# ParBLiSS/FastANI

Hardware: NVIDIA H100
Metric: genome-pairs/sec (many-to-many, k=16, fragLen=3000) (higher is better)
Workload: dtype u64

## Files before the change

### fastani_b200/csrc/capi.cu

```cuda
#include "common.cuh"
#include <algorithm>
#include <cstring>
#include <cstdlib>

struct bani_ctx    { bani::Ctx c; };
struct bani_genome { bani::Genome g; };
struct bani_index  { bani::Index *ix; };
struct bani_qsketch { bani::QSketch *qs; };

namespace bani {
static thread_local std::string g_err;
void set_last_error(const std::string &m) { g_err = m; }
const char *const PATH_NAMES[NPATH] = {
  "l1.class0", "l1.class1", "l1.class2", "l1.class3", "l1.class4", "l1.class5", "l1.class6", "l1.class7", "l1.class8",
  "l1.class9", "l1.class10", "l1.class11", "l1.class12", "l1.device_wide",
  "lookup.walk_saturated", "lookup.walk_full_bucket",
  "l2.events_nt64", "l2.events_nt128", "l2.events_nt256", "l2.dir1024", "l2.dir4096", "l2.staged", "l2.direct",
  "l2.exact_at_bounds", "l2.exact_total",
  "piece.mapped", "piece.split_hits", "piece.split_events", "cgi.passes", "cgi.sparse"};
}

using namespace bani;

#define BANI_TRY try {
#define BANI_CATCH } catch (const bani::Error &e) { bani::set_last_error(e.what()); return e.code; } \
  catch (const std::bad_alloc &) { bani::set_last_error("host allocation failed"); return BANI_ERR_NOMEM; } \
  catch (const std::exception &e) { bani::set_last_error(e.what()); return BANI_ERR_INTERNAL; }

template <typename T>
static T *host_copy(const std::vector<T> &v)
{
  if (v.empty()) return nullptr;
  T *p = (T *)malloc(sizeof(T) * v.size());
// ... 72 lines not shown
  c->c.prm = *p;
  if (c->c.prm.kmer_size < 1 || c->c.prm.kmer_size > 32) fail(BANI_ERR_LIMIT, "k-mer size %d outside [1, 32]", c->c.prm.kmer_size);
  if (c->c.prm.frag_len < 1) fail(BANI_ERR_ARG, "fragment length must be positive");
  if (c->c.prm.window_size <= 0)
    c->c.prm.window_size = stat_recommended_window_size(p->p_value, p->kmer_size, p->perc_identity, p->frag_len, p->reference_size);
  cudaDeviceProp prop;
  BANI_CUDA(cudaGetDeviceProperties(&prop, device));
  c->c.smCount = prop.multiProcessorCount;
  c->c.memTotal = prop.totalGlobalMem;
  {
    CtxFlags &f = c->c.flags;
    if (getenv("BANI_NO_SKETCH_REUSE")) f.sketchReuse = 0;
    if (const char *e = getenv("BANI_MAX_HITS_PER_PIECE")) f.maxHitsPerPiece = std::max(1ll, atoll(e));
    if (const char *e = getenv("BANI_FRAG_L1_MAX")) f.fragL1Max = std::max(0ll, atoll(e));
    if (const char *e = getenv("BANI_L2_STAGE")) f.l2Stage = atoi(e) != 0;
    if (const char *e = getenv("BANI_TRACE")) f.trace = atoi(e) != 0;
    if (const char *e = getenv("BANI_L2E_BUCKETS")) { const int v = atoi(e); if (v == 1024 || v == 4096) f.l2eBuckets = v; }
    if (const char *e = getenv("BANI_CGI_SPARSE")) {
      const std::string v(e);
      if (v == "-1") f.cgiSparse = -1;
      else if (v == "0") f.cgiSparse = 0;
      else if (v == "1") f.cgiSparse = 1;
      else fail(BANI_ERR_ARG, "BANI_CGI_SPARSE=%s is not -1 (chosen per piece), 0 (dense) or 1 (sparse)", e);
    }
    uint64_t b = 0;
    if (const char *e = getenv("BANI_INDEX_BUDGET")) {
      if (!parse_byte_count(e, &b)) fail(BANI_ERR_ARG, "BANI_INDEX_BUDGET=%s is not a byte count (digits, optionally followed by K, M or G)", e);
      f.indexBytesBudget = b;
    }
    if (const char *e = getenv("BANI_QUERY_BUDGET")) {
// ... 40 lines not shown
  return BANI_OK;
  BANI_CATCH
}

int bani_ctx_set_flag(bani_ctx *ctx, const char *name, int64_t value)
{
  BANI_TRY
  if (!ctx || !name) fail(BANI_ERR_ARG, "null argument");
  CtxFlags &f = ctx->c.flags;
  const std::string n(name);
  if (n == "sketch_reuse") f.sketchReuse = value != 0;
  else if (n == "max_hits_per_piece") { if (value < 1) fail(BANI_ERR_ARG, "max_hits_per_piece must be positive"); f.maxHitsPerPiece = value; }
  else if (n == "frag_l1_max") { if (value < 0) fail(BANI_ERR_ARG, "frag_l1_max must not be negative"); f.fragL1Max = value; }
  else if (n == "l2e_buckets") { if (value != 0 && value != 1024 && value != 4096) fail(BANI_ERR_ARG, "l2e_buckets must be 0, 1024 or 4096"); f.l2eBuckets = (int)value; }
  else if (n == "l2_stage") f.l2Stage = value != 0;
  else if (n == "upload_group_words") { if (value < 1) fail(BANI_ERR_ARG, "upload_group_words must be positive"); f.uploadGroupWords = value; }
  else if (n == "frags_per_piece") { if (value < 1 || value > (1ll << 18)) fail(BANI_ERR_ARG, "frags_per_piece must be in [1, 2^18]"); f.fragsPerPiece = value; }
  else if (n == "event_bytes_per_piece") { if (value < 0) fail(BANI_ERR_ARG, "event_bytes_per_piece must not be negative"); f.eventBytesPerPiece = value; }
  else if (n == "cgi_table_queries") { if (value < 0) fail(BANI_ERR_ARG, "cgi_table_queries must not be negative"); f.cgiTableQueries = value; }
  else if (n == "l2_fast") f.l2Fast = value != 0;
  else if (n == "count_paths") f.countPaths = value != 0;
  else if (n == "cgi_sparse") { if (value < -1 || value > 1) fail(BANI_ERR_ARG, "cgi_sparse must be -1, 0 or 1"); f.cgiSparse = (int)value; }
  else if (n == "index_bytes_budget") { if (value < 0) fail(BANI_ERR_ARG, "index_bytes_budget must not be negative"); f.indexBytesBudget = (unsigned long long)value; }
  else if (n == "query_sketch_budget") { if (value < 0) fail(BANI_ERR_ARG, "query_sketch_budget must not be negative"); f.querySketchBudget = (unsigned long long)value; }
  else fail(BANI_ERR_ARG, "unknown flag '%s'", name);
  return BANI_OK;
  BANI_CATCH
}

int bani_ctx_path_counts(bani_ctx *ctx, char (*names)[32], uint64_t *counts, int32_t n_max, int32_t *n)
// ... 694 lines not shown
```

### fastani_b200/csrc/common.cuh

```cuda
#pragma once
#include <cuda_runtime.h>
#include <stdint.h>
#include <string>
#include <vector>
#include <memory>
#include <map>
#include <stdexcept>
#include <cstdio>
#include <cstdarg>
#include <chrono>
#include "../../include/fastani_b200.h"

namespace bani {

struct Error : std::runtime_error {
  int code;
  Error(int c, const std::string &m) : std::runtime_error(m), code(c) {}
};

void set_last_error(const std::string &m);

[[noreturn]] inline void fail(int code, const char *fmt, ...)
{
  char buf[512];
// ... 135 lines not shown
};

template <typename T>
struct View {
  T *p = nullptr; size_t n = 0;
  size_t bytes() const { return n * sizeof(T); }
  void release() {}
};

struct CtxFlags {
  int sketchReuse = 1;
  long long maxHitsPerPiece = 3ll << 29;
  long long fragL1Max = 8192;
  int l2eBuckets = 0;
  int trace = 0;
  int l2Stage = 1;
  long long uploadGroupWords = 16ll << 20;
  long long fragsPerPiece = 1ll << 18;
  long long eventBytesPerPiece = 0;
  long long cgiTableQueries = 0;
  int l2Fast = 1;
  int countPaths = 0;
  int cgiSparse = -1;
  unsigned long long indexBytesBudget = 0;
  unsigned long long querySketchBudget = 0;
};

enum PathId {
  P_L1_CLASS0 = 0, P_L1_DEVICE_WIDE = 13,
  P_LOOKUP_WALK_SATURATED, P_LOOKUP_WALK_FULL_BUCKET,
  P_L2_EVENTS_NT64, P_L2_EVENTS_NT128, P_L2_EVENTS_NT256, P_L2_DIR1024, P_L2_DIR4096, P_L2_STAGED, P_L2_DIRECT,
  P_L2_EXACT_AT_BOUNDS, P_L2_EXACT_TOTAL,
  P_PIECE_MAPPED, P_PIECE_SPLIT_HITS, P_PIECE_SPLIT_EVENTS, P_CGI_PASSES, P_CGI_SPARSE,
  NPATH
};
extern const char *const PATH_NAMES[NPATH];

struct Ctx {
  int device = 0;
  cudaStream_t stream = nullptr;
  cudaStream_t copyStream = nullptr;
  bani_params prm{};
  CtxFlags flags;
  int smCount = 0;
  size_t memTotal = 0;
  StatLut lut;
  DevBuf<int32_t> d_minHits; DevBuf<uint32_t> d_rowOff; DevBuf<float> d_ident, d_upper;
// ... 130 lines not shown
void qsketch_map(Ctx *ctx, const Index *ix, const QSketch *const *sketches, int32_t nSketches,
                 bool wantRows, bool wantCgi, MapOutput &out, bool wantFrags = false);

static constexpr unsigned long long FRAG_L1_MAX = 8192;
static constexpr int FRAG_NCLASS = 13;
static_assert(P_L1_DEVICE_WIDE == FRAG_NCLASS, "one path counter per L1 size class");
__host__ __device__ inline int frag_class_items(int cls)
{
  return cls < 8 ? cls + 1 : (cls == 8 ? 10 : cls == 9 ? 12 : cls == 10 ? 16 : cls == 11 ? 24 : 32);
}
struct FragL1Args {
  const uint32_t *segStart; const int32_t *sCount; int32_t F;
  const uint32_t *hitLo, *hitCnt; const unsigned long long *hitOff;
  const uint32_t *posIdx; const int2 *recPos;
  const int32_t *minHits; int fragLen, keyBits;
  int32_t *stSeq, *stStart, *stEnd;
  uint32_t *candCount;
};
void frag_classify(Ctx *ctx, const uint32_t *segStart, const unsigned long long *hitOff, int32_t F,
                   uint32_t *candCount, uint32_t *fragClass, uint32_t *classCount, uint32_t *classList, unsigned long long maxFast);
void frag_l1_fast(Ctx *ctx, const FragL1Args &a, const uint32_t *classList, const uint32_t *classCount);
void cand_stage(Ctx *ctx, const int32_t *cFrag, const int32_t *cSeq, const int32_t *cStart, const int32_t *cEnd, uint32_t C,
                const uint32_t *segStart, const unsigned long long *hitOff, int32_t *stSeq, int32_t *stStart, int32_t *stEnd,
                uint32_t *candCount);
void cand_compact(Ctx *ctx, const uint32_t *segStart, const unsigned long long *hitOff, int32_t F,
                  const uint32_t *candCount, const uint32_t *candOff, const int32_t *stSeq, const int32_t *stStart,
                  const int32_t *stEnd, int32_t *cFrag, int32_t *cSeq, int32_t *cStart, int32_t *cEnd);

void synth_genome(Ctx *ctx, uint64_t seed, uint32_t ancestor, uint32_t strain, uint32_t ppm,
                  int64_t len, uint8_t *hostOut);

size_t cub_sort_pairs_u32_temp(size_t n);
void   cub_sort_pairs_u32(void *temp, size_t tempBytes, const uint32_t *kin, uint32_t *kout,
                          const uint32_t *vin, uint32_t *vout, size_t n, int endBit, cudaStream_t s);
size_t cub_sort_keys_u64_temp(size_t n);
void   cub_sort_keys_u64(void *temp, size_t tempBytes, const uint64_t *kin, uint64_t *kout, size_t n,
                         int beginBit, int endBit, cudaStream_t s);
size_t cub_sort_pairs_u64_u32_temp(size_t n);
void   cub_sort_pairs_u64_u32(void *temp, size_t tempBytes, const uint64_t *kin, uint64_t *kout,
                              const uint32_t *vin, uint32_t *vout, size_t n, int endBit, cudaStream_t s);
size_t cub_scan_u32_temp(size_t n);
void   cub_exclusive_sum_u32(void *temp, size_t tempBytes, const uint32_t *in, uint32_t *out, size_t n, cudaStream_t s);
// ... 5 lines not shown
```

### fastani_b200/csrc/hits.cu

```cuda
#define BANI_FILE_TAG 1
#include "common.cuh"

namespace bani {

static inline unsigned nblk(uint64_t n, int t = 256) { return (unsigned)((n + t - 1) / t); }

__global__ void frag_classify_kernel(const uint32_t *segStart, const unsigned long long *hitOff, int32_t F,
                                     uint32_t *candCount, uint32_t *fragClass, uint32_t *classCount, uint32_t *classList, unsigned long long maxFast)
{
  const int f = blockIdx.x * blockDim.x + threadIdx.x;
  if (f >= F) return;
  const unsigned long long n = hitOff[segStart[f + 1]] - hitOff[segStart[f]];
  candCount[f] = 0;
  uint32_t cls = FRAG_NCLASS + 1;
  if (n > maxFast) cls = FRAG_NCLASS;
  else if (n > 0) { cls = 0; while (n > 256ull * (unsigned long long)frag_class_items(cls)) cls++; }
  fragClass[f] = cls;
  if (cls <= FRAG_NCLASS) { const uint32_t o = atomicAdd(&classCount[cls], 1u); if (cls < FRAG_NCLASS) classList[(size_t)cls * F + o] = (uint32_t)f; }
}

template <int ITEMS, int DB>
__device__ __forceinline__ uint32_t *block_radix_sort(uint32_t *in, uint32_t *out, uint16_t *hist ,
                                                       uint32_t *digitBase , uint32_t *wsum , int keyBits)
{
// ... 84 lines not shown
  const uint32_t *sorted = block_radix_sort<ITEMS, DB>(bufA, bufB, hist, digitBase, wsum, a.keyBits);
  uint32_t keys[ITEMS];
#pragma unroll
  for (int i = 0; i < ITEMS; i++) keys[i] = sorted[i * 256 + tid];
  __syncthreads();
  int32_t *s_w = reinterpret_cast<int32_t *>(bufA), *s_seq = reinterpret_cast<int32_t *>(bufB);
#pragma unroll
  for (int i = 0; i < ITEMS; i++) {
    const int r = i * 256 + tid;
    if (r < n) { const int2 p = __ldg(&a.recPos[keys[i]]); s_w[r] = p.x; s_seq[r] = p.y; }
  }
  __syncthreads();
  const int mh = a.minHits[s];
  uint32_t *qualW = reinterpret_cast<uint32_t *>(hist);
  uint16_t *slice = reinterpret_cast<uint16_t *>(qualW + ITEMS * 8);
  int32_t starts[ITEMS];
  uint32_t qualMask = 0;
#pragma unroll
  for (int i = 0; i < ITEMS; i++) {
    const int r = i * 256 + tid, rb = r + mh - 1;
    bool q = false;
    starts[i] = 0;
    if (rb < n && s_seq[rb] == s_seq[r]) {
      const int32_t wb = s_w[rb];
      if (wb - s_w[r] < a.fragLen) { q = true; starts[i] = max(0, wb - a.fragLen + 1); }
    }
    const uint32_t bal = __ballot_sync(0xffffffffu, q);
    if (lane == 0) qualW[i * 8 + wid] = bal;
    if (q) qualMask |= 1u << i;
  }
  __syncthreads();
  auto qual_at = [&](int r) -> bool { return (qualW[r >> 5] >> (r & 31)) & 1u; };
  auto start_at = [&](int r) -> int32_t { return max(0, s_w[r + mh - 1] - a.fragLen + 1); };
  uint32_t headMask = 0, tailMask = 0;
  uint32_t headBallot[ITEMS];
#pragma unroll
  for (int i = 0; i < ITEMS; i++) {
    const int r = i * 256 + tid;
    bool hd = false;
    if ((qualMask >> i) & 1u) {
      const int32_t st = starts[i];
      const bool merged = r > 0 && s_seq[r - 1] == s_seq[r] && qual_at(r - 1) && s_w[r - 1] >= st;
      const bool nextMerges = r + 1 < n && s_seq[r + 1] == s_seq[r] && qual_at(r + 1) && s_w[r] >= start_at(r + 1);
      hd = !merged;
      if (hd) headMask |= 1u << i;
      if (!nextMerges) tailMask |= 1u << i;
    }
    headBallot[i] = __ballot_sync(0xffffffffu, hd);
    if (lane == 0) slice[i * 8 + wid] = (uint16_t)__popc(headBallot[i]);
  }
  __syncthreads();
  uint32_t total = 0;
  {
    uint32_t run = 0;
#pragma unroll
    for (int i = 0; i < ITEMS; i++) {
      uint32_t before = run;
#pragma unroll
      for (int ww = 0; ww < 8; ww++) { const uint32_t c = slice[i * 8 + ww]; if (ww < wid) before += c; run += c; }
      const uint32_t hb = headBallot[i];
      const uint32_t upto = before + __popc(hb & ((2u << lane) - 1u));
      const int r = i * 256 + tid;
      if ((headMask >> i) & 1u) { a.stSeq[base + upto - 1] = s_seq[r]; a.stStart[base + upto - 1] = starts[i]; }
      if ((tailMask >> i) & 1u) a.stEnd[base + upto - 1] = s_w[r];
    }
    total = run;
  }
  if (tid == 0) a.candCount[f] = total;
}

template <int CAPW>
__global__ void __launch_bounds__(128)
frag_l1_warp_kernel(const FragL1Args a, const uint32_t *list, uint32_t count)
{
  __shared__ uint32_t sm[4][3 * CAPW];
  const int lane = threadIdx.x & 31, wid = threadIdx.x >> 5;
  const uint32_t slot = blockIdx.x * 4 + wid;
  if (slot >= count) return;
  const int f = (int)list[slot];
// ... 36 lines not shown
  for (int r0 = 0; r0 < n; r0 += 32) {
    const uint32_t qNext = __ballot_sync(0xffffffffu, qual(r0 + 32 + lane));
    const int r = r0 + lane;
    bool hd = false, tl = false;
    int32_t st = 0;
    if ((qCur >> lane) & 1u) {
      st = start_of(r);
      const bool qL = lane ? ((qCur >> (lane - 1)) & 1u) : ((qPrev >> 31) & 1u);
      const bool qR = lane < 31 ? ((qCur >> (lane + 1)) & 1u) : (qNext & 1u);
      const bool merged = r > 0 && qL && s_seq[r - 1] == s_seq[r] && s_w[r - 1] >= st;
      const bool nextMerges = r + 1 < n && qR && s_seq[r + 1] == s_seq[r] && s_w[r] >= start_of(r + 1);
      hd = !merged; tl = !nextMerges;
    }
    const uint32_t hb = __ballot_sync(0xffffffffu, hd);
    const uint32_t upto = run + __popc(hb & ((2u << lane) - 1u));
    if (hd) { a.stSeq[base + upto - 1] = s_seq[r]; a.stStart[base + upto - 1] = st; }
    if (tl) a.stEnd[base + upto - 1] = s_w[r];
    run += __popc(hb);
    qPrev = qCur; qCur = qNext;
  }
  if (lane == 0) a.candCount[f] = run;
}

template <int ITEMS>
static void launch_class(Ctx *ctx, const FragL1Args &a, const uint32_t *list, uint32_t count, cudaStream_t st)
{
  if (count == 0) return;
  constexpr int ND = 1 << FragSortBits<ITEMS>::DB;
  const size_t shm = sizeof(uint32_t) * 2 * 256 * ITEMS + 2 * 8 * ND + 4 * ND + 64;
  if (ctx->first_time((const void *)frag_l1_kernel<ITEMS>))
    BANI_CUDA(cudaFuncSetAttribute(frag_l1_kernel<ITEMS>, cudaFuncAttributeMaxDynamicSharedMemorySize, (int)shm));
  frag_l1_kernel<ITEMS><<<count, 256, shm, st>>>(a, list, count);
// ... 17 lines not shown
  launch_class<3>(ctx, a, classList + 2 * F, classCount[2], st);
  launch_class<4>(ctx, a, classList + 3 * F, classCount[3], st);
  launch_class<5>(ctx, a, classList + 4 * F, classCount[4], st);
  launch_class<6>(ctx, a, classList + 5 * F, classCount[5], st);
  launch_class<7>(ctx, a, classList + 6 * F, classCount[6], st);
  launch_class<8>(ctx, a, classList + 7 * F, classCount[7], st);
  launch_class<10>(ctx, a, classList + 8 * F, classCount[8], st);
  launch_class<12>(ctx, a, classList + 9 * F, classCount[9], st);
  launch_class<16>(ctx, a, classList + 10 * F, classCount[10], st);
  launch_class<24>(ctx, a, classList + 11 * F, classCount[11], st);
  launch_class<32>(ctx, a, classList + 12 * F, classCount[12], st);
  for (int i = 0; i < FRAG_NCLASS; i++) if (classCount[i]) ctx->launches++;
  BANI_CUDA(cudaGetLastError());
}

__global__ void cand_stage_kernel(const int32_t *cFrag, const int32_t *cSeq, const int32_t *cStart, const int32_t *cEnd, uint32_t C,
                                  const uint32_t *segStart, const unsigned long long *hitOff,
                                  int32_t *stSeq, int32_t *stStart, int32_t *stEnd, uint32_t *candCount)
{
  const uint32_t c = blockIdx.x * blockDim.x + threadIdx.x;
  if (c >= C) return;
  const int f = cFrag[c];
  uint32_t lo = 0, hi = c;
  while (lo < hi) { uint32_t mid = (lo + hi) >> 1; if (cFrag[mid] < f) lo = mid + 1; else hi = mid; }
  const unsigned long long o = hitOff[segStart[f]] + (c - lo);
  stSeq[o] = cSeq[c]; stStart[o] = cStart[c]; stEnd[o] = cEnd[c];
  atomicAdd(&candCount[f], 1u);
}

void cand_stage(Ctx *ctx, const int32_t *cFrag, const int32_t *cSeq, const int32_t *cStart, const int32_t *cEnd, uint32_t C,
                const uint32_t *segStart, const unsigned long long *hitOff, int32_t *stSeq, int32_t *stStart, int32_t *stEnd,
                uint32_t *candCount)
{
  if (!C) return;
  cand_stage_kernel<<<nblk(C), 256, 0, ctx->stream>>>(cFrag, cSeq, cStart, cEnd, C, segStart, hitOff, stSeq, stStart, stEnd, candCount);
  ctx->launches++;
}

__global__ void cand_compact_kernel(const uint32_t *segStart, const unsigned long long *hitOff, int32_t F,
                                    const uint32_t *candCount, const uint32_t *candOff,
                                    const int32_t *stSeq, const int32_t *stStart, const int32_t *stEnd,
                                    int32_t *cFrag, int32_t *cSeq, int32_t *cStart, int32_t *cEnd)
{
  const int f = (int)((blockIdx.x * (unsigned)blockDim.x + threadIdx.x) >> 5), lane = threadIdx.x & 31;
  if (f >= F) return;
  const uint32_t n = candCount[f];
  if (!n) return;
  const unsigned long long src = hitOff[segStart[f]];
  const uint32_t dst = candOff[f];
  for (uint32_t i = lane; i < n; i += 32) {
    cFrag[dst + i] = f; cSeq[dst + i] = stSeq[src + i]; cStart[dst + i] = stStart[src + i]; cEnd[dst + i] = stEnd[src + i];
  }
}

void cand_compact(Ctx *ctx, const uint32_t *segStart, const unsigned long long *hitOff, int32_t F,
                  const uint32_t *candCount, const uint32_t *candOff, const int32_t *stSeq, const int32_t *stStart,
                  const int32_t *stEnd, int32_t *cFrag, int32_t *cSeq, int32_t *cStart, int32_t *cEnd)
{
  cand_compact_kernel<<<nblk((uint64_t)F * 32), 256, 0, ctx->stream>>>(segStart, hitOff, F, candCount, candOff, stSeq, stStart, stEnd,
                                                                         cFrag, cSeq, cStart, cEnd);
  ctx->launches++;
}

}
```

### fastani_b200/csrc/map.cu

```cuda
#include "common.cuh"
#include "cgi_rows.hpp"
#include <algorithm>
#include <cstring>
#include <deque>

namespace bani {

static inline unsigned nblk(uint64_t n, int t = 256) { return (unsigned)((n + t - 1) / t); }

static constexpr int SU_THREADS = 128;
static constexpr int SU_CAP = 4096;

__global__ void __launch_bounds__(SU_THREADS)
sort_unique_kernel(uint32_t *fragHash, const uint32_t *segStart, int32_t F, int32_t *sCount,
                   int *smax, int *err, int minN )
{
  __shared__ uint32_t a[SU_CAP];
  __shared__ uint32_t wsum[SU_THREADS / 32];
  const int f = blockIdx.x, tid = threadIdx.x;
  const uint32_t beg = segStart[f];
  const int n = (int)(segStart[f + 1] - beg);
  if (n <= minN) return;
  if (n > SU_CAP) { if (tid == 0) { atomicExch(err, 1); sCount[f] = 0; } return; }
  if (n == 0) { if (tid == 0) sCount[f] = 0; return; }
// ... 169 lines not shown
  }
  if (!nextMerges) fl |= 2;
  return fl;
}

__global__ void l1_flag_kernel(const L1Args a, uint32_t *head)
{
  unsigned long long i = (unsigned long long)blockIdx.x * blockDim.x + threadIdx.x;
  if (i > a.N) return;
  if (i == a.N) { head[i] = 0; return; }
  int32_t start; uint32_t ra; int f;
  head[i] = l1_flags(a, i, start, ra, f) & 1u;
}

__global__ void l1_write_kernel(const L1Args a, const uint32_t *head, const uint32_t *headScan,
                                int32_t *cFrag, int32_t *cSeq, int32_t *cStart, int32_t *cEnd)
{
  unsigned long long i = (unsigned long long)blockIdx.x * blockDim.x + threadIdx.x;
  if (i >= a.N) return;
  int32_t start; uint32_t ra; int f;
  const uint32_t fl = l1_flags(a, i, start, ra, f);
  if (fl & 1) { const uint32_t c = headScan[i]; cFrag[c] = f; cSeq[c] = a.recSeq[ra]; cStart[c] = start; }
  if (fl & 2) { const uint32_t c = headScan[i] + head[i] - 1; cEnd[c] = a.recWpos[ra]; }
}

struct L2Args {
  const int32_t *cFrag, *cSeq, *cStart, *cEnd; uint32_t C;
  const uint32_t *fragHash; const uint32_t *segStart; const int32_t *sCount;
  const uint32_t *recHash; const int32_t *recWpos; const uint32_t *recLink; const uint32_t *contigRecOff;
  int fragLen, cmw, smax;
  uint8_t *scratch; size_t stride;
  int32_t *cPos, *cBest;
  int onlyFlagged;
};

__device__ __forceinline__ uint32_t lb_wpos(const int32_t *wpos, uint32_t lo, uint32_t hi, int32_t v)
{
  while (lo < hi) { uint32_t mid = (lo + hi) >> 1; if (wpos[mid] < v) lo = mid + 1; else hi = mid; }
// ... 60 lines not shown
    a.cBest[c] = best;
  }
}

static constexpr int L2_SMAX = 2047;
static constexpr int L2_SHM_BUDGET = 200 * 1024;
static constexpr uint32_t EV_M = 1u, EV_D = 2u, EV_S = 4u, EV_JMASK = 0xFFE0u;
__host__ __device__ __forceinline__ uint32_t ev_rank(uint32_t j) { return j << 5; }

static constexpr int L2E_RING = 1024;
static constexpr int L2E_FLUSH_IT = 4;
static constexpr int L2E_BF_MAX = L2E_RING - 64 * L2E_FLUSH_IT - 96;

struct L2PArgs {
  const int32_t *cFrag, *cSeq, *cStart, *cEnd; uint32_t C;
  const uint32_t *fragCandOff;
  const uint32_t *fragHash; const uint32_t *segStart; const int32_t *sCount;
  const uint4 *rec; const int32_t *recWposSoA; const uint32_t *contigRecOff;
  const uint2 *rec8; const uint32_t *recLink; const uint32_t *blkMax;
  int fragLen, cmw, sLimit, shiftA, nBuckets;
  int stage;
  uint32_t *cB0, *cE0, *cLast, *cNEv, *cChunks;
  uint16_t *cMB;
  const uint32_t *cOff;
  const unsigned long long *grpOff;
  uint16_t *events;
  const uint32_t *perm; uint32_t warpBytes;
  int32_t *cPos, *cBest; unsigned long long *ctr_n2;
};

__global__ void frag_cand_off_kernel(const int32_t *cFrag, uint32_t C, int32_t F, uint32_t *fragCandOff)
{
  int f = blockIdx.x * blockDim.x + threadIdx.x;
  if (f > F) return;
  uint32_t lo = 0, hi = C;
  while (lo < hi) { uint32_t mid = (lo + hi) >> 1; if (cFrag[mid] < f) lo = mid + 1; else hi = mid; }
  fragCandOff[f] = lo;
}

__device__ __forceinline__ int32_t rec_wpos(const uint4 *rec, uint32_t i) { return (int32_t)(__ldg(&rec[i].y) & 0x7FFFFFFFu); }
__device__ __forceinline__ uint32_t lb_rec(const uint4 *rec, uint32_t lo, uint32_t hi, int32_t v)
{
  while (lo < hi) { uint32_t mid = (lo + hi) >> 1; if (rec_wpos(rec, mid) < v) lo = mid + 1; else hi = mid; }
  return lo;
}

__global__ void l2_bounds_kernel(const L2PArgs a)
{
  const uint32_t c = blockIdx.x * blockDim.x + threadIdx.x;
  unsigned long long n2 = 0;
  if (c < a.C) {
    const int seq = a.cSeq[c];
    const uint32_t lo = a.contigRecOff[seq], hi = a.contigRecOff[seq + 1];
    const uint32_t b0 = lb_wpos(a.recWposSoA, lo, hi, a.cStart[c]);
    const uint32_t e0 = lb_wpos(a.recWposSoA, b0, hi, __ldg(&a.recWposSoA[b0]) + a.cmw);
    const uint32_t last = lb_wpos(a.recWposSoA, b0, hi, a.cEnd[c] + a.fragLen);
    n2 = last - b0;
    const int s = a.sCount[a.cFrag[c]];
    uint32_t nEv = 0;
    if (e0 < last) {
      const uint32_t back = __ldg(&a.rec[last - 1].w) & 0xFFFFu;
      const uint32_t bEnd = (back > last - 1 - b0) ? b0 : last - 1 - back;
      nEv = (e0 - b0) + (last - e0) + (bEnd - b0);
    }
    a.cB0[c] = b0; a.cE0[c] = e0; a.cLast[c] = last;
    const bool fast = s >= 1 && s <= a.sLimit && nEv < (1u << 20);
    {
      uint32_t mbk = 0, mfw = 0;
      if (fast && nEv) {
        const uint32_t blk1 = (last - 1) >> 10;
        for (uint32_t blk = b0 >> 10; blk <= blk1 && mbk != 0xFFFFu; blk++) { const uint32_t v = __ldg(&a.blkMax[blk]); mbk = max(mbk, v & 0xFFFFu); mfw = max(mfw, v >> 16); }
      }
      a.cMB[c] = (uint16_t)((a.stage && mbk + mfw <= (uint32_t)L2E_BF_MAX) ? mbk : 0xFFFFu);
    }
    a.cNEv[c] = fast ? nEv : 0u;
    a.cChunks[c] = fast ? (nEv + 15) >> 4 : 0u;
    a.cBest[c] = (fast || nEv == 0) ? 0 : -1;
    a.cPos[c] = 0;
  } else if (c == a.C) a.cChunks[c] = 0;
  for (int o = 16; o; o >>= 1) n2 += __shfl_xor_sync(0xffffffffu, n2, o);
  if ((threadIdx.x & 31) == 0 && n2) atomicAdd(a.ctr_n2, n2);
}

__global__ void l2_sortkey_kernel(const uint32_t *cNEv, uint32_t C, uint32_t *key, uint32_t *val)
{
  const uint32_t c = blockIdx.x * blockDim.x + threadIdx.x;
  if (c >= C) return;
  key[c] = 0xFFFFFu - min(cNEv[c], 0xFFFFFu);
  val[c] = c;
}

__global__ void l2_group_steps_kernel(const uint32_t *cChunks, const uint32_t *perm, uint32_t C, uint32_t nGrp, uint32_t *grpSteps)
{
  const uint32_t G = blockIdx.x * blockDim.x + threadIdx.x;
  if (G > nGrp) return;
  grpSteps[G] = G < nGrp ? cChunks[perm[G * 32]] : 0u;
// ... 1085 lines not shown
        unsigned long long N = 0;
        BANI_CUDA(cudaMemcpyAsync(&N, hitOff.p + T, 8, cudaMemcpyDeviceToHost, st));
        if (countPaths) BANI_CUDA(cudaMemcpyAsync(pp + P_LOOKUP_WALK_SATURATED, walkCtr.p, 16, cudaMemcpyDeviceToHost, st));
        BANI_CUDA(cudaStreamSynchronize(st));
        ctx->mark("piece: lookup done");
        if (N > maxHits && nQc > 1) split_in_halves(P_PIECE_SPLIT_HITS);
        if (!split && N > 0xfffffff0ull) fail(BANI_ERR_LIMIT, "one query genome gathers more than 2^32 index hits");
        if (!split) out.ctr.hits += N;

        if (N > 0 && !split) {
          BANI_SCRATCH(uint32_t, candCount, (size_t)F + 1);
          BANI_SCRATCH(uint32_t, candOff, (size_t)F + 1);
          BANI_SCRATCH(uint32_t, fragClass, F);
          BANI_SCRATCH(uint32_t, classList, (size_t)FRAG_NCLASS * F);
          BANI_SCRATCH(uint32_t, classCount, FRAG_NCLASS + 2);
          BANI_SCRATCH(int32_t, stSeq, N);
          BANI_SCRATCH(int32_t, stStart, N);
          BANI_SCRATCH(int32_t, stEnd, N);
          const long long maxFast = std::max(0ll, std::min(ctx->flags.fragL1Max, (long long)FRAG_L1_MAX));
          uint32_t hClass[FRAG_NCLASS + 2];
          { Stage sg(ctx, "frag_l1", 12.0 * N);
            frag_classify(ctx, segStart.p, hitOff.p, F, candCount.p, fragClass.p, classCount.p, classList.p, (unsigned long long)maxFast);
            BANI_CUDA(cudaMemcpyAsync(hClass, classCount.p, sizeof hClass, cudaMemcpyDeviceToHost, st));
            BANI_CUDA(cudaStreamSynchronize(st));
            for (int i = 0; i <= FRAG_NCLASS; i++) pp[P_L1_CLASS0 + i] += hClass[i];
            FragL1Args fa; fa.segStart = segStart.p; fa.sCount = sCount.p; fa.F = F; fa.hitLo = hitLo.p; fa.hitCnt = hitCnt.p; fa.hitOff = hitOff.p;
            fa.posIdx = ix->posIdx.p; fa.recPos = ix->pos8.p; fa.minHits = ctx->d_minHits.p; fa.fragLen = fragLen;
            fa.keyBits = 1; while (fa.keyBits < 32 && (1ull << fa.keyBits) < ix->M) fa.keyBits++;
            fa.stSeq = stSeq.p; fa.stStart = stStart.p; fa.stEnd = stEnd.p; fa.candCount = candCount.p;
            frag_l1_fast(ctx, fa, classList.p, hClass); }
          if (hClass[FRAG_NCLASS] > 0) {
            BANI_SCRATCH(uint32_t, bigCnt, T + 1);
            BANI_SCRATCH(unsigned long long, bigOff, T + 1);
            mask_hits_kernel<<<nblk(T + 1), 256, 0, st>>>(segStart.p, F, (uint32_t)T, hitCnt.p, fragClass.p, bigCnt.p); ctx->launches++;
            { size_t tb = cub_scan_u64_temp(T + 1);
              BANI_SCRATCH(uint8_t, tmp, tb);
              cub_exclusive_sum_u32_to_u64(tmp.p, tb, bigCnt.p, (uint64_t *)bigOff.p, T + 1, st); }
            unsigned long long NB = 0;
            BANI_CUDA(cudaMemcpyAsync(&NB, bigOff.p + T, 8, cudaMemcpyDeviceToHost, st));
            BANI_CUDA(cudaStreamSynchronize(st));
            BANI_SCRATCH(unsigned long long, keysA, NB);
            BANI_SCRATCH(unsigned long long, keysB, NB);
            { Stage sg(ctx, "hit_gather", 12.0 * NB);
              gather_kernel<<<nblk(T), 256, 0, st>>>(segStart.p, F, (uint32_t)T, hitLo.p, bigCnt.p, bigOff.p, ix->posIdx.p, keysA.p); ctx->launches++; }
// ... 5 lines not shown
            L1Args la; la.keys = keysB.p; la.N = NB; la.segStart = segStart.p; la.hitOff = bigOff.p; la.sCount = sCount.p;
            la.minHits = ctx->d_minHits.p; la.recSeq = ix->seqId.p; la.recWpos = ix->wpos.p; la.fragLen = fragLen;
            BANI_SCRATCH(uint32_t, head, NB + 1);
            BANI_SCRATCH(uint32_t, headScan, NB + 1);
            { Stage sg(ctx, "l1_flags", 8.0 * NB);
              l1_flag_kernel<<<nblk(NB + 1), 256, 0, st>>>(la, head.p);
              ctx->launches++;
              size_t tb = cub_scan_u32_temp(NB + 1);
              BANI_SCRATCH(uint8_t, tmp, tb);
              cub_exclusive_sum_u32(tmp.p, tb, head.p, headScan.p, NB + 1, st); }
            uint32_t CB = 0;
            BANI_CUDA(cudaMemcpyAsync(&CB, headScan.p + NB, 4, cudaMemcpyDeviceToHost, st));
            BANI_CUDA(cudaStreamSynchronize(st));
            if (CB > 0) {
              BANI_SCRATCH(int32_t, bFrag, CB);
              BANI_SCRATCH(int32_t, bSeq, CB);
              BANI_SCRATCH(int32_t, bStart, CB);
              BANI_SCRATCH(int32_t, bEnd, CB);
              Stage sg(ctx, "l1_write", 8.0 * NB);
              l1_write_kernel<<<nblk(NB), 256, 0, st>>>(la, head.p, headScan.p, bFrag.p, bSeq.p, bStart.p, bEnd.p); ctx->launches++;
              cand_stage(ctx, bFrag.p, bSeq.p, bStart.p, bEnd.p, CB, segStart.p, hitOff.p, stSeq.p, stStart.p, stEnd.p, candCount.p);
            }
          }
          { size_t tb = cub_scan_u32_temp((size_t)F + 1);
            BANI_SCRATCH(uint8_t, tmp, tb);
            BANI_CUDA(cudaMemsetAsync(candCount.p + F, 0, 4, st));
            cub_exclusive_sum_u32(tmp.p, tb, candCount.p, candOff.p, (size_t)F + 1, st); }
          uint32_t C = 0;
          BANI_CUDA(cudaMemcpyAsync(&C, candOff.p + F, 4, cudaMemcpyDeviceToHost, st));
          BANI_CUDA(cudaStreamSynchronize(st));
          out.ctr.candidates += C;

          if (C > 0) {
            BANI_SCRATCH(int32_t, cFrag, C);
            BANI_SCRATCH(int32_t, cSeq, C);
            BANI_SCRATCH(int32_t, cStart, C);
            BANI_SCRATCH(int32_t, cEnd, C);
            BANI_SCRATCH(int32_t, cPos, C);
            BANI_SCRATCH(int32_t, cBest, C);
            cand_compact(ctx, segStart.p, hitOff.p, F, candCount.p, candOff.p, stSeq.p, stStart.p, stEnd.p, cFrag.p, cSeq.p, cStart.p, cEnd.p);

            L2Args l2; l2.cFrag = cFrag.p; l2.cSeq = cSeq.p; l2.cStart = cStart.p; l2.cEnd = cEnd.p; l2.C = C;
            l2.fragHash = fragHash.p; l2.segStart = segStart.p; l2.sCount = sCount.p;
            l2.recHash = ix->hash.p; l2.recWpos = ix->wpos.p; l2.recLink = ix->link.p; l2.contigRecOff = ix->contigRecOff.p;
            l2.fragLen = fragLen; l2.cmw = cmw; l2.smax = smax;
            l2.stride = ((size_t)2 * (smax + 2) + smax + 15) / 16 * 16;
            const unsigned blocks = (unsigned)std::min<uint64_t>((C + 63) / 64, (uint64_t)ctx->smCount * 16);
            BANI_SCRATCH(uint8_t, scratch, (size_t)blocks * 64 * l2.stride);
            BANI_SCRATCH(unsigned long long, d_n2, 1);
            BANI_CUDA(cudaMemsetAsync(d_n2.p, 0, 8, st));
            l2.scratch = scratch.p; l2.cPos = cPos.p; l2.cBest = cBest.p; l2.onlyFlagged = 1;
            size_t idEv = (size_t)-1; double evBytes = 0;
            {
              unsigned long long totalSteps = 0;
              Stage sgb(ctx, "l2_bounds", 12.0 * C);
              BANI_SCRATCH(uint32_t, fragCandOff, (size_t)F + 1);
              frag_cand_off_kernel<<<nblk((uint64_t)F + 1), 256, 0, st>>>(cFrag.p, C, F, fragCandOff.p);
              ctx->launches++;
              L2PArgs lp; lp.cFrag = cFrag.p; lp.cSeq = cSeq.p; lp.cStart = cStart.p; lp.cEnd = cEnd.p; lp.C = C;
              lp.fragCandOff = fragCandOff.p; lp.fragHash = fragHash.p; lp.segStart = segStart.p; lp.sCount = sCount.p;
              lp.rec = ix->rec.p; lp.recWposSoA = ix->wpos.p; lp.contigRecOff = ix->contigRecOff.p; lp.fragLen = fragLen; lp.cmw = cmw;
              lp.rec8 = ix->rec8.p; lp.recLink = ix->link.p; lp.blkMax = ix->blkMax.p; lp.stage = ctx->flags.l2Stage;
              lp.sLimit = (ctx->flags.l2Fast && cmw >= 2 && ix->cmw == cmw && ix->rec8.p) ? std::min(std::min(smax, L2_SMAX), L2_SHM_BUDGET / (L2S_WARPS * 32) - 2) : 0;
              lp.nBuckets = ((uint64_t)C >= 8ull * (uint64_t)F) ? L2E_BUCKETS : 1024;
              { const int forced = ctx->flags.l2eBuckets;
                if (forced == 1024 || forced == L2E_BUCKETS) lp.nBuckets = forced; }
              { int sh = lp.nBuckets == L2E_BUCKETS ? 20 : 22; while (sh > 8 && ((uint64_t)std::max(smax, 1) * (uint64_t)w << sh) > ((1ull << 32) * (uint64_t)(L2E_BUCKETS / lp.nBuckets))) sh--; lp.shiftA = sh; }
              lp.warpBytes = (uint32_t)(std::max(lp.sLimit, 1) + 1) * 32u;
              BANI_SCRATCH(uint32_t, cB0, C);
              BANI_SCRATCH(uint32_t, cE0, C);
              BANI_SCRATCH(uint32_t, cLast, C);
              BANI_SCRATCH(uint32_t, cNEv, C);
              BANI_SCRATCH(uint32_t, cChunks, (size_t)C + 1);
              BANI_SCRATCH(uint32_t, cOff, (size_t)C + 1);
              BANI_SCRATCH(uint16_t, cMB, (size_t)C + 1);
              lp.cMB = cMB.p;
              lp.cB0 = cB0.p; lp.cE0 = cE0.p; lp.cLast = cLast.p; lp.cNEv = cNEv.p; lp.cChunks = cChunks.p; lp.cOff = cOff.p;
              lp.cPos = cPos.p; lp.cBest = cBest.p; lp.ctr_n2 = d_n2.p; lp.events = nullptr; lp.perm = nullptr;
              l2_bounds_kernel<<<nblk((uint64_t)C + 1), 256, 0, st>>>(lp); ctx->launches++;
              if (countPaths) pp[P_L2_EXACT_AT_BOUNDS] += count_exact(ctx, cBest.p, C);
              if (lp.sLimit > 0) {
                BANI_SCRATCH(uint32_t, skey, C);
                BANI_SCRATCH(uint32_t, skey2, C);
                BANI_SCRATCH(uint32_t, sval, C);
                BANI_SCRATCH(uint32_t, perm, C);
                l2_sortkey_kernel<<<nblk(C), 256, 0, st>>>(cNEv.p, C, skey.p, sval.p); ctx->launches++;
                { size_t tb = cub_sort_pairs_u32_temp(C);
                  BANI_SCRATCH(uint8_t, tmp, tb);
                  cub_sort_pairs_u32(tmp.p, tb, skey.p, skey2.p, sval.p, perm.p, C, 20, st); }
                lp.perm = perm.p;
                const uint32_t nGrp = (C + 31) / 32;
                BANI_SCRATCH(uint32_t, grpSteps, (size_t)nGrp + 1);
                BANI_SCRATCH(unsigned long long, grpOff, (size_t)nGrp + 1);
                l2_group_steps_kernel<<<nblk((uint64_t)nGrp + 1), 256, 0, st>>>(cChunks.p, perm.p, C, nGrp, grpSteps.p); ctx->launches++;
                { size_t tb = cub_scan_u64_temp((size_t)nGrp + 1);
// ... 239 lines not shown
```

Baseline: 2.114 million.

## Seed L2 bound searches from L1 record indices via galloping search

Level-1 candidate staging now carries the head and tail record indices in place of the sequence id and end window position. Those are resolved through recPos during compaction. The L2 bounds kernel uses the record indices, plus a density estimate from the window size, as hints for exponential (galloping) lower-bound searches, replacing binary searches over the whole contig range. This is meant to cut global memory probes per candidate in l2_bounds, at the cost of extra rec loads, a gather in compaction, and more scratch arrays. Optional path counters check that the hinted bounds match the exact ones.

```diff
diff --git a/fastani_b200/csrc/capi.cu b/fastani_b200/csrc/capi.cu
--- a/fastani_b200/csrc/capi.cu
+++ b/fastani_b200/csrc/capi.cu
@@ -16,7 +16,7 @@
   "l1.class9", "l1.class10", "l1.class11", "l1.class12", "l1.device_wide",
   "lookup.walk_saturated", "lookup.walk_full_bucket",
   "l2.events_nt64", "l2.events_nt128", "l2.events_nt256", "l2.dir1024", "l2.dir4096", "l2.staged", "l2.direct",
-  "l2.exact_at_bounds", "l2.exact_total",
+  "l2.exact_at_bounds", "l2.exact_total", "l2.bounds_hint", "l2.bounds_contig", "l2.bounds_hint_differs",
   "piece.mapped", "piece.split_hits", "piece.split_events", "cgi.passes", "cgi.sparse"};
 }
 
@@ -119,6 +119,7 @@
     if (const char *e = getenv("BANI_MAX_HITS_PER_PIECE")) f.maxHitsPerPiece = std::max(1ll, atoll(e));
     if (const char *e = getenv("BANI_FRAG_L1_MAX")) f.fragL1Max = std::max(0ll, atoll(e));
     if (const char *e = getenv("BANI_L2_STAGE")) f.l2Stage = atoi(e) != 0;
+    if (const char *e = getenv("BANI_L2_BOUNDS_HINT")) f.l2BoundsHint = atoi(e) != 0;
     if (const char *e = getenv("BANI_TRACE")) f.trace = atoi(e) != 0;
     if (const char *e = getenv("BANI_L2E_BUCKETS")) { const int v = atoi(e); if (v == 1024 || v == 4096) f.l2eBuckets = v; }
     if (const char *e = getenv("BANI_CGI_SPARSE")) {
@@ -189,6 +190,7 @@
   else if (n == "frag_l1_max") { if (value < 0) fail(BANI_ERR_ARG, "frag_l1_max must not be negative"); f.fragL1Max = value; }
   else if (n == "l2e_buckets") { if (value != 0 && value != 1024 && value != 4096) fail(BANI_ERR_ARG, "l2e_buckets must be 0, 1024 or 4096"); f.l2eBuckets = (int)value; }
   else if (n == "l2_stage") f.l2Stage = value != 0;
+  else if (n == "l2_bounds_hint") f.l2BoundsHint = value != 0;
   else if (n == "upload_group_words") { if (value < 1) fail(BANI_ERR_ARG, "upload_group_words must be positive"); f.uploadGroupWords = value; }
   else if (n == "frags_per_piece") { if (value < 1 || value > (1ll << 18)) fail(BANI_ERR_ARG, "frags_per_piece must be in [1, 2^18]"); f.fragsPerPiece = value; }
   else if (n == "event_bytes_per_piece") { if (value < 0) fail(BANI_ERR_ARG, "event_bytes_per_piece must not be negative"); f.eventBytesPerPiece = value; }
diff --git a/fastani_b200/csrc/common.cuh b/fastani_b200/csrc/common.cuh
--- a/fastani_b200/csrc/common.cuh
+++ b/fastani_b200/csrc/common.cuh
@@ -173,6 +173,7 @@
   long long fragL1Max = 8192;
   int l2eBuckets = 0;
   int trace = 0;
+  int l2BoundsHint = 1;
   int l2Stage = 1;
   long long uploadGroupWords = 16ll << 20;
   long long fragsPerPiece = 1ll << 18;
@@ -189,7 +190,7 @@
   P_L1_CLASS0 = 0, P_L1_DEVICE_WIDE = 13,
   P_LOOKUP_WALK_SATURATED, P_LOOKUP_WALK_FULL_BUCKET,
   P_L2_EVENTS_NT64, P_L2_EVENTS_NT128, P_L2_EVENTS_NT256, P_L2_DIR1024, P_L2_DIR4096, P_L2_STAGED, P_L2_DIRECT,
-  P_L2_EXACT_AT_BOUNDS, P_L2_EXACT_TOTAL,
+  P_L2_EXACT_AT_BOUNDS, P_L2_EXACT_TOTAL, P_L2_BOUNDS_HINT, P_L2_BOUNDS_CONTIG, P_L2_BOUNDS_HINT_DIFFERS,
   P_PIECE_MAPPED, P_PIECE_SPLIT_HITS, P_PIECE_SPLIT_EVENTS, P_CGI_PASSES, P_CGI_SPARSE,
   NPATH
 };
@@ -350,18 +351,19 @@
   const uint32_t *hitLo, *hitCnt; const unsigned long long *hitOff;
   const uint32_t *posIdx; const int2 *recPos;
   const int32_t *minHits; int fragLen, keyBits;
-  int32_t *stSeq, *stStart, *stEnd;
+  uint32_t *stRecH; int32_t *stStart; uint32_t *stRecT;
   uint32_t *candCount;
 };
 void frag_classify(Ctx *ctx, const uint32_t *segStart, const unsigned long long *hitOff, int32_t F,
                    uint32_t *candCount, uint32_t *fragClass, uint32_t *classCount, uint32_t *classList, unsigned long long maxFast);
 void frag_l1_fast(Ctx *ctx, const FragL1Args &a, const uint32_t *classList, const uint32_t *classCount);
-void cand_stage(Ctx *ctx, const int32_t *cFrag, const int32_t *cSeq, const int32_t *cStart, const int32_t *cEnd, uint32_t C,
-                const uint32_t *segStart, const unsigned long long *hitOff, int32_t *stSeq, int32_t *stStart, int32_t *stEnd,
+void cand_stage(Ctx *ctx, const int32_t *cFrag, const uint32_t *cRecH, const int32_t *cStart, const uint32_t *cRecT, uint32_t C,
+                const uint32_t *segStart, const unsigned long long *hitOff, uint32_t *stRecH, int32_t *stStart, uint32_t *stRecT,
                 uint32_t *candCount);
 void cand_compact(Ctx *ctx, const uint32_t *segStart, const unsigned long long *hitOff, int32_t F,
-                  const uint32_t *candCount, const uint32_t *candOff, const int32_t *stSeq, const int32_t *stStart,
-                  const int32_t *stEnd, int32_t *cFrag, int32_t *cSeq, int32_t *cStart, int32_t *cEnd);
+                  const uint32_t *candCount, const uint32_t *candOff, const uint32_t *stRecH, const int32_t *stStart,
+                  const uint32_t *stRecT, const int2 *recPos, int32_t *cFrag, int32_t *cSeq, int32_t *cStart, int32_t *cEnd,
+                  uint32_t *cRecH, uint32_t *cRecT);
 
 void synth_genome(Ctx *ctx, uint64_t seed, uint32_t ancestor, uint32_t strain, uint32_t ppm,
                   int64_t len, uint8_t *hostOut);
diff --git a/fastani_b200/csrc/hits.cu b/fastani_b200/csrc/hits.cu
--- a/fastani_b200/csrc/hits.cu
+++ b/fastani_b200/csrc/hits.cu
@@ -122,16 +122,14 @@
   const int mh = a.minHits[s];
   uint32_t *qualW = reinterpret_cast<uint32_t *>(hist);
   uint16_t *slice = reinterpret_cast<uint16_t *>(qualW + ITEMS * 8);
-  int32_t starts[ITEMS];
   uint32_t qualMask = 0;
 #pragma unroll
   for (int i = 0; i < ITEMS; i++) {
     const int r = i * 256 + tid, rb = r + mh - 1;
     bool q = false;
-    starts[i] = 0;
     if (rb < n && s_seq[rb] == s_seq[r]) {
       const int32_t wb = s_w[rb];
-      if (wb - s_w[r] < a.fragLen) { q = true; starts[i] = max(0, wb - a.fragLen + 1); }
+      if (wb - s_w[r] < a.fragLen) q = true;
     }
     const uint32_t bal = __ballot_sync(0xffffffffu, q);
     if (lane == 0) qualW[i * 8 + wid] = bal;
@@ -147,7 +145,7 @@
     const int r = i * 256 + tid;
     bool hd = false;
     if ((qualMask >> i) & 1u) {
-      const int32_t st = starts[i];
+      const int32_t st = start_at(r);
       const bool merged = r > 0 && s_seq[r - 1] == s_seq[r] && qual_at(r - 1) && s_w[r - 1] >= st;
       const bool nextMerges = r + 1 < n && s_seq[r + 1] == s_seq[r] && qual_at(r + 1) && s_w[r] >= start_at(r + 1);
       hd = !merged;
@@ -169,8 +167,8 @@
       const uint32_t hb = headBallot[i];
       const uint32_t upto = before + __popc(hb & ((2u << lane) - 1u));
       const int r = i * 256 + tid;
-      if ((headMask >> i) & 1u) { a.stSeq[base + upto - 1] = s_seq[r]; a.stStart[base + upto - 1] = starts[i]; }
-      if ((tailMask >> i) & 1u) a.stEnd[base + upto - 1] = s_w[r];
+      if ((headMask >> i) & 1u) { a.stRecH[base + upto - 1] = keys[i]; a.stStart[base + upto - 1] = start_at(r); }
+      if ((tailMask >> i) & 1u) a.stRecT[base + upto - 1] = keys[i];
     }
     total = run;
   }
@@ -237,8 +235,8 @@
     }
     const uint32_t hb = __ballot_sync(0xffffffffu, hd);
     const uint32_t upto = run + __popc(hb & ((2u << lane) - 1u));
-    if (hd) { a.stSeq[base + upto - 1] = s_seq[r]; a.stStart[base + upto - 1] = st; }
-    if (tl) a.stEnd[base + upto - 1] = s_w[r];
+    if (hd) { a.stRecH[base + upto - 1] = keys[r]; a.stStart[base + upto - 1] = st; }
+    if (tl) a.stRecT[base + upto - 1] = keys[r];
     run += __popc(hb);
     qPrev = qCur; qCur = qNext;
   }
@@ -286,9 +284,9 @@
   BANI_CUDA(cudaGetLastError());
 }
 
-__global__ void cand_stage_kernel(const int32_t *cFrag, const int32_t *cSeq, const int32_t *cStart, const int32_t *cEnd, uint32_t C,
+__global__ void cand_stage_kernel(const int32_t *cFrag, const uint32_t *cRecH, const int32_t *cStart, const uint32_t *cRecT, uint32_t C,
                                   const uint32_t *segStart, const unsigned long long *hitOff,
-                                  int32_t *stSeq, int32_t *stStart, int32_t *stEnd, uint32_t *candCount)
+                                  uint32_t *stRecH, int32_t *stStart, uint32_t *stRecT, uint32_t *candCount)
 {
   const uint32_t c = blockIdx.x * blockDim.x + threadIdx.x;
   if (c >= C) return;
@@ -296,23 +294,23 @@
   uint32_t lo = 0, hi = c;
   while (lo < hi) { uint32_t mid = (lo + hi) >> 1; if (cFrag[mid] < f) lo = mid + 1; else hi = mid; }
   const unsigned long long o = hitOff[segStart[f]] + (c - lo);
-  stSeq[o] = cSeq[c]; stStart[o] = cStart[c]; stEnd[o] = cEnd[c];
+  stRecH[o] = cRecH[c]; stStart[o] = cStart[c]; stRecT[o] = cRecT[c];
   atomicAdd(&candCount[f], 1u);
 }
 
-void cand_stage(Ctx *ctx, const int32_t *cFrag, const int32_t *cSeq, const int32_t *cStart, const int32_t *cEnd, uint32_t C,
-                const uint32_t *segStart, const unsigned long long *hitOff, int32_t *stSeq, int32_t *stStart, int32_t *stEnd,
+void cand_stage(Ctx *ctx, const int32_t *cFrag, const uint32_t *cRecH, const int32_t *cStart, const uint32_t *cRecT, uint32_t C,
+                const uint32_t *segStart, const unsigned long long *hitOff, uint32_t *stRecH, int32_t *stStart, uint32_t *stRecT,
                 uint32_t *candCount)
 {
   if (!C) return;
-  cand_stage_kernel<<<nblk(C), 256, 0, ctx->stream>>>(cFrag, cSeq, cStart, cEnd, C, segStart, hitOff, stSeq, stStart, stEnd, candCount);
+  cand_stage_kernel<<<nblk(C), 256, 0, ctx->stream>>>(cFrag, cRecH, cStart, cRecT, C, segStart, hitOff, stRecH, stStart, stRecT, candCount);
   ctx->launches++;
 }
 
 __global__ void cand_compact_kernel(const uint32_t *segStart, const unsigned long long *hitOff, int32_t F,
                                     const uint32_t *candCount, const uint32_t *candOff,
-                                    const int32_t *stSeq, const int32_t *stStart, const int32_t *stEnd,
-                                    int32_t *cFrag, int32_t *cSeq, int32_t *cStart, int32_t *cEnd)
+                                    const uint32_t *stRecH, const int32_t *stStart, const uint32_t *stRecT, const int2 *recPos,
+                                    int32_t *cFrag, int32_t *cSeq, int32_t *cStart, int32_t *cEnd, uint32_t *cRecH, uint32_t *cRecT)
 {
   const int f = (int)((blockIdx.x * (unsigned)blockDim.x + threadIdx.x) >> 5), lane = threadIdx.x & 31;
   if (f >= F) return;
@@ -321,16 +319,19 @@
   const unsigned long long src = hitOff[segStart[f]];
   const uint32_t dst = candOff[f];
   for (uint32_t i = lane; i < n; i += 32) {
-    cFrag[dst + i] = f; cSeq[dst + i] = stSeq[src + i]; cStart[dst + i] = stStart[src + i]; cEnd[dst + i] = stEnd[src + i];
+    const uint32_t rh = stRecH[src + i], rt = stRecT[src + i];
+    cFrag[dst + i] = f; cSeq[dst + i] = __ldg(&recPos[rh].y); cStart[dst + i] = stStart[src + i]; cEnd[dst + i] = __ldg(&recPos[rt].x);
+    cRecH[dst + i] = rh; cRecT[dst + i] = rt;
   }
 }
 
 void cand_compact(Ctx *ctx, const uint32_t *segStart, const unsigned long long *hitOff, int32_t F,
-                  const uint32_t *candCount, const uint32_t *candOff, const int32_t *stSeq, const int32_t *stStart,
-                  const int32_t *stEnd, int32_t *cFrag, int32_t *cSeq, int32_t *cStart, int32_t *cEnd)
-{
-  cand_compact_kernel<<<nblk((uint64_t)F * 32), 256, 0, ctx->stream>>>(segStart, hitOff, F, candCount, candOff, stSeq, stStart, stEnd,
-                                                                         cFrag, cSeq, cStart, cEnd);
+                  const uint32_t *candCount, const uint32_t *candOff, const uint32_t *stRecH, const int32_t *stStart,
+                  const uint32_t *stRecT, const int2 *recPos, int32_t *cFrag, int32_t *cSeq, int32_t *cStart, int32_t *cEnd,
+                  uint32_t *cRecH, uint32_t *cRecT)
+{
+  cand_compact_kernel<<<nblk((uint64_t)F * 32), 256, 0, ctx->stream>>>(segStart, hitOff, F, candCount, candOff, stRecH, stStart, stRecT,
+                                                                         recPos, cFrag, cSeq, cStart, cEnd, cRecH, cRecT);
   ctx->launches++;
 }
 
diff --git a/fastani_b200/csrc/map.cu b/fastani_b200/csrc/map.cu
--- a/fastani_b200/csrc/map.cu
+++ b/fastani_b200/csrc/map.cu
@@ -207,14 +207,14 @@
 }
 
 __global__ void l1_write_kernel(const L1Args a, const uint32_t *head, const uint32_t *headScan,
-                                int32_t *cFrag, int32_t *cSeq, int32_t *cStart, int32_t *cEnd)
+                                int32_t *cFrag, uint32_t *cRecH, int32_t *cStart, uint32_t *cRecT)
 {
   unsigned long long i = (unsigned long long)blockIdx.x * blockDim.x + threadIdx.x;
   if (i >= a.N) return;
   int32_t start; uint32_t ra; int f;
   const uint32_t fl = l1_flags(a, i, start, ra, f);
-  if (fl & 1) { const uint32_t c = headScan[i]; cFrag[c] = f; cSeq[c] = a.recSeq[ra]; cStart[c] = start; }
-  if (fl & 2) { const uint32_t c = headScan[i] + head[i] - 1; cEnd[c] = a.recWpos[ra]; }
+  if (fl & 1) { const uint32_t c = headScan[i]; cFrag[c] = f; cRecH[c] = ra; cStart[c] = start; }
+  if (fl & 2) { const uint32_t c = headScan[i] + head[i] - 1; cRecT[c] = ra; }
 }
 
 struct L2Args {
@@ -305,11 +305,14 @@
 
 struct L2PArgs {
   const int32_t *cFrag, *cSeq, *cStart, *cEnd; uint32_t C;
+  const uint32_t *cRecH, *cRecT;
+  int boundsHint;
+  unsigned long long *ctr_bounds;
   const uint32_t *fragCandOff;
   const uint32_t *fragHash; const uint32_t *segStart; const int32_t *sCount;
   const uint4 *rec; const int32_t *recWposSoA; const uint32_t *contigRecOff;
   const uint2 *rec8; const uint32_t *recLink; const uint32_t *blkMax;
-  int fragLen, cmw, sLimit, shiftA, nBuckets;
+  int fragLen, cmw, w, sLimit, shiftA, nBuckets;
   int stage;
   uint32_t *cB0, *cE0, *cLast, *cNEv, *cChunks;
   uint16_t *cMB;
@@ -336,16 +339,56 @@
   return lo;
 }
 
+__device__ __forceinline__ uint32_t lb_wpos_from(const int32_t *wpos, uint32_t lo, uint32_t hi, int32_t v, uint32_t h)
+{
+  if (lo >= hi) return lo;
+  h = min(max(h, lo), hi - 1);
+  uint32_t p = h, step = 1;
+  if (__ldg(&wpos[h]) < v) {
+    for (;;) {
+      const uint32_t q = p + step;
+      if (q >= hi || __ldg(&wpos[q]) >= v) return lb_wpos(wpos, p + 1, min(q, hi), v);
+      p = q; step <<= 1;
+    }
+  }
+  for (;;) {
+    if (p - lo < step) return lb_wpos(wpos, lo, p, v);
+    const uint32_t q = p - step;
+    if (__ldg(&wpos[q]) < v) return lb_wpos(wpos, q + 1, p, v);
+    p = q; step <<= 1;
+  }
+}
+
 __global__ void l2_bounds_kernel(const L2PArgs a)
 {
   const uint32_t c = blockIdx.x * blockDim.x + threadIdx.x;
   unsigned long long n2 = 0;
+  bool differs = false;
   if (c < a.C) {
     const int seq = a.cSeq[c];
     const uint32_t lo = a.contigRecOff[seq], hi = a.contigRecOff[seq + 1];
-    const uint32_t b0 = lb_wpos(a.recWposSoA, lo, hi, a.cStart[c]);
-    const uint32_t e0 = lb_wpos(a.recWposSoA, b0, hi, __ldg(&a.recWposSoA[b0]) + a.cmw);
-    const uint32_t last = lb_wpos(a.recWposSoA, b0, hi, a.cEnd[c] + a.fragLen);
+    const int32_t vb = a.cStart[c], vl = a.cEnd[c] + a.fragLen;
+    uint32_t b0, e0, last;
+    if (a.boundsHint) {
+      const uint32_t h = a.cRecH[c], t = a.cRecT[c];
+      const uint4 rh = __ldg(&a.rec[h]);
+      const uint32_t p = h + 1 - min(rh.w & 0xFFFFu, h + 1);
+      const long long dpos = (long long)vb - ((long long)(rh.y & 0x7FFFFFFFu) - a.cmw + 2);
+      const long long gb = (long long)p + dpos * 2 / (a.w + 1);
+      const uint32_t fwdT = __ldg(&a.rec[t].w) >> 16;
+      b0 = lb_wpos_from(a.recWposSoA, lo, hi, vb, (uint32_t)min(max(gb, (long long)lo), (long long)hi));
+      const uint32_t fwdB = b0 < hi ? __ldg(&a.rec[b0].w) >> 16 : 0u;
+      e0 = lb_wpos_from(a.recWposSoA, b0, hi, __ldg(&a.recWposSoA[b0]) + a.cmw, (uint32_t)min((unsigned long long)b0 + fwdB, (unsigned long long)hi));
+      last = lb_wpos_from(a.recWposSoA, b0, hi, vl, (uint32_t)min((unsigned long long)t + fwdT, (unsigned long long)hi));
+    } else {
+      b0 = lb_wpos(a.recWposSoA, lo, hi, vb);
+      e0 = lb_wpos(a.recWposSoA, b0, hi, __ldg(&a.recWposSoA[b0]) + a.cmw);
+      last = lb_wpos(a.recWposSoA, b0, hi, vl);
+    }
+    if (a.ctr_bounds && a.boundsHint) {
+      const uint32_t b = lb_wpos(a.recWposSoA, lo, hi, vb);
+      differs = b != b0 || lb_wpos(a.recWposSoA, b, hi, __ldg(&a.recWposSoA[b]) + a.cmw) != e0 || lb_wpos(a.recWposSoA, b, hi, vl) != last;
+    }
     n2 = last - b0;
     const int s = a.sCount[a.cFrag[c]];
     uint32_t nEv = 0;
@@ -371,6 +414,13 @@
   } else if (c == a.C) a.cChunks[c] = 0;
   for (int o = 16; o; o >>= 1) n2 += __shfl_xor_sync(0xffffffffu, n2, o);
   if ((threadIdx.x & 31) == 0 && n2) atomicAdd(a.ctr_n2, n2);
+  if (a.ctr_bounds) {
+    const uint32_t nc = __popc(__ballot_sync(0xffffffffu, c < a.C)), nd = __popc(__ballot_sync(0xffffffffu, differs));
+    if ((threadIdx.x & 31) == 0) {
+      if (nc) atomicAdd(&a.ctr_bounds[a.boundsHint ? 0 : 1], (unsigned long long)nc);
+      if (nd) atomicAdd(&a.ctr_bounds[2], (unsigned long long)nd);
+    }
+  }
 }
 
 __global__ void l2_sortkey_kernel(const uint32_t *cNEv, uint32_t C, uint32_t *key, uint32_t *val)
@@ -1486,9 +1536,9 @@
           BANI_SCRATCH(uint32_t, fragClass, F);
           BANI_SCRATCH(uint32_t, classList, (size_t)FRAG_NCLASS * F);
           BANI_SCRATCH(uint32_t, classCount, FRAG_NCLASS + 2);
-          BANI_SCRATCH(int32_t, stSeq, N);
+          BANI_SCRATCH(uint32_t, stRecH, N);
           BANI_SCRATCH(int32_t, stStart, N);
-          BANI_SCRATCH(int32_t, stEnd, N);
+          BANI_SCRATCH(uint32_t, stRecT, N);
           const long long maxFast = std::max(0ll, std::min(ctx->flags.fragL1Max, (long long)FRAG_L1_MAX));
           uint32_t hClass[FRAG_NCLASS + 2];
           { Stage sg(ctx, "frag_l1", 12.0 * N);
@@ -1499,7 +1549,7 @@
             FragL1Args fa; fa.segStart = segStart.p; fa.sCount = sCount.p; fa.F = F; fa.hitLo = hitLo.p; fa.hitCnt = hitCnt.p; fa.hitOff = hitOff.p;
             fa.posIdx = ix->posIdx.p; fa.recPos = ix->pos8.p; fa.minHits = ctx->d_minHits.p; fa.fragLen = fragLen;
             fa.keyBits = 1; while (fa.keyBits < 32 && (1ull << fa.keyBits) < ix->M) fa.keyBits++;
-            fa.stSeq = stSeq.p; fa.stStart = stStart.p; fa.stEnd = stEnd.p; fa.candCount = candCount.p;
+            fa.stRecH = stRecH.p; fa.stStart = stStart.p; fa.stRecT = stRecT.p; fa.candCount = candCount.p;
             frag_l1_fast(ctx, fa, classList.p, hClass); }
           if (hClass[FRAG_NCLASS] > 0) {
             BANI_SCRATCH(uint32_t, bigCnt, T + 1);
@@ -1535,12 +1585,12 @@
             BANI_CUDA(cudaStreamSynchronize(st));
             if (CB > 0) {
               BANI_SCRATCH(int32_t, bFrag, CB);
-              BANI_SCRATCH(int32_t, bSeq, CB);
+              BANI_SCRATCH(uint32_t, bRecH, CB);
               BANI_SCRATCH(int32_t, bStart, CB);
-              BANI_SCRATCH(int32_t, bEnd, CB);
+              BANI_SCRATCH(uint32_t, bRecT, CB);
               Stage sg(ctx, "l1_write", 8.0 * NB);
-              l1_write_kernel<<<nblk(NB), 256, 0, st>>>(la, head.p, headScan.p, bFrag.p, bSeq.p, bStart.p, bEnd.p); ctx->launches++;
-              cand_stage(ctx, bFrag.p, bSeq.p, bStart.p, bEnd.p, CB, segStart.p, hitOff.p, stSeq.p, stStart.p, stEnd.p, candCount.p);
+              l1_write_kernel<<<nblk(NB), 256, 0, st>>>(la, head.p, headScan.p, bFrag.p, bRecH.p, bStart.p, bRecT.p); ctx->launches++;
+              cand_stage(ctx, bFrag.p, bRecH.p, bStart.p, bRecT.p, CB, segStart.p, hitOff.p, stRecH.p, stStart.p, stRecT.p, candCount.p);
             }
           }
           { size_t tb = cub_scan_u32_temp((size_t)F + 1);
@@ -1559,7 +1609,10 @@
             BANI_SCRATCH(int32_t, cEnd, C);
             BANI_SCRATCH(int32_t, cPos, C);
             BANI_SCRATCH(int32_t, cBest, C);
-            cand_compact(ctx, segStart.p, hitOff.p, F, candCount.p, candOff.p, stSeq.p, stStart.p, stEnd.p, cFrag.p, cSeq.p, cStart.p, cEnd.p);
+            BANI_SCRATCH(uint32_t, cRecH, C);
+            BANI_SCRATCH(uint32_t, cRecT, C);
+            cand_compact(ctx, segStart.p, hitOff.p, F, candCount.p, candOff.p, stRecH.p, stStart.p, stRecT.p, ix->pos8.p,
+                         cFrag.p, cSeq.p, cStart.p, cEnd.p, cRecH.p, cRecT.p);
 
             L2Args l2; l2.cFrag = cFrag.p; l2.cSeq = cSeq.p; l2.cStart = cStart.p; l2.cEnd = cEnd.p; l2.C = C;
             l2.fragHash = fragHash.p; l2.segStart = segStart.p; l2.sCount = sCount.p;
@@ -1580,8 +1633,9 @@
               ctx->launches++;
               L2PArgs lp; lp.cFrag = cFrag.p; lp.cSeq = cSeq.p; lp.cStart = cStart.p; lp.cEnd = cEnd.p; lp.C = C;
               lp.fragCandOff = fragCandOff.p; lp.fragHash = fragHash.p; lp.segStart = segStart.p; lp.sCount = sCount.p;
-              lp.rec = ix->rec.p; lp.recWposSoA = ix->wpos.p; lp.contigRecOff = ix->contigRecOff.p; lp.fragLen = fragLen; lp.cmw = cmw;
+              lp.rec = ix->rec.p; lp.recWposSoA = ix->wpos.p; lp.contigRecOff = ix->contigRecOff.p; lp.fragLen = fragLen; lp.cmw = cmw; lp.w = w;
               lp.rec8 = ix->rec8.p; lp.recLink = ix->link.p; lp.blkMax = ix->blkMax.p; lp.stage = ctx->flags.l2Stage;
+              lp.cRecH = cRecH.p; lp.cRecT = cRecT.p; lp.boundsHint = ctx->flags.l2BoundsHint;
               lp.sLimit = (ctx->flags.l2Fast && cmw >= 2 && ix->cmw == cmw && ix->rec8.p) ? std::min(std::min(smax, L2_SMAX), L2_SHM_BUDGET / (L2S_WARPS * 32) - 2) : 0;
               lp.nBuckets = ((uint64_t)C >= 8ull * (uint64_t)F) ? L2E_BUCKETS : 1024;
               { const int forced = ctx->flags.l2eBuckets;
@@ -1598,8 +1652,17 @@
               lp.cMB = cMB.p;
               lp.cB0 = cB0.p; lp.cE0 = cE0.p; lp.cLast = cLast.p; lp.cNEv = cNEv.p; lp.cChunks = cChunks.p; lp.cOff = cOff.p;
               lp.cPos = cPos.p; lp.cBest = cBest.p; lp.ctr_n2 = d_n2.p; lp.events = nullptr; lp.perm = nullptr;
+              DevBuf<unsigned long long> boundsCtr;
+              lp.ctr_bounds = nullptr;
+              if (countPaths) { boundsCtr.alloc(3, st); BANI_CUDA(cudaMemsetAsync(boundsCtr.p, 0, 24, st)); lp.ctr_bounds = boundsCtr.p; }
               l2_bounds_kernel<<<nblk((uint64_t)C + 1), 256, 0, st>>>(lp); ctx->launches++;
-              if (countPaths) pp[P_L2_EXACT_AT_BOUNDS] += count_exact(ctx, cBest.p, C);
+              if (countPaths) {
+                pp[P_L2_EXACT_AT_BOUNDS] += count_exact(ctx, cBest.p, C);
+                unsigned long long bc[3];
+                BANI_CUDA(cudaMemcpyAsync(bc, boundsCtr.p, sizeof bc, cudaMemcpyDeviceToHost, st));
+                BANI_CUDA(cudaStreamSynchronize(st));
+                pp[P_L2_BOUNDS_HINT] += bc[0]; pp[P_L2_BOUNDS_CONTIG] += bc[1]; pp[P_L2_BOUNDS_HINT_DIFFERS] += bc[2];
+              }
               if (lp.sLimit > 0) {
                 BANI_SCRATCH(uint32_t, skey, C);
                 BANI_SCRATCH(uint32_t, skey2, C);
```

Result: faster. 2.170 million, median of 6 (+2.7%).
